# GitHubOfAndrew/TeAMOFlow

Hardware: AMD Instinct MI355X
Metric: train_interactions_per_sec (higher is better)
Workload: dtype f32

## Files before the change

### include/tmf.h

```cpp
#ifndef TMF_H
#define TMF_H

#include <stddef.h>
#include <stdint.h>

#ifdef __cplusplus
extern "C" {
#endif

#define TMF_VERSION 203

#define TMF_OK 0
#define TMF_E_INVALID (-1)
#define TMF_E_LAUNCH (-2)
#define TMF_E_UNSUPPORTED (-3)

#define TMF_EPI_ADAM 0
#define TMF_EPI_GRAD 1

int tmf_version(void);
const char* tmf_last_error(void);

int tmf_padded_ld(int n_components);

// ... 83 lines not shown
    const int64_t* rowptr;
    const int32_t* col;
    const int32_t* pos_off;
    int32_t n_users, n_samples, n_slices;
    int32_t slice_begin, slice_count, item_base;
    int32_t flags;
    int32_t n_items;
} tmf_slice_lists;
#define TMF_SLICE_XCD_MAJOR 1
#define TMF_SLICE_N_ITEMS_STATED 2
int tmf_wmrb_scores3_f32(const tmf_slice_lists* lists, const void* U, const void* V, float* sp, float* p,
                         int n_components, void* stream);
int tmf_wmrb_scores3_bf16(const tmf_slice_lists* lists, const void* U, const void* V, float* sp, float* p,
                          int n_components, void* stream);
int tmf_wmrb_scores5_users_per_workgroup(void);
int tmf_wmrb_scores5_supported(int n_components, int bf16, int64_t n_items);
size_t tmf_wmrb_scores5_workspace_bytes(int64_t n_wg, int32_t n_windows, int wgs_per_launch);
int tmf_wmrb_scores5_f32(const int32_t* ids, const int32_t* outs, const int64_t* wg_ptr, int64_t n_wg, int64_t n_users,
                         int64_t n_items, const void* U, const void* V, float* sp, float* p, int n_components,
                         int wgs_per_launch, const int32_t* wstart, int32_t n_windows, int lag, void* workspace,
                         size_t workspace_bytes, void* stream);
int tmf_wmrb_scores5_bf16(const int32_t* ids, const int32_t* outs, const int64_t* wg_ptr, int64_t n_wg, int64_t n_users,
                          int64_t n_items, const void* U, const void* V, float* sp, float* p, int n_components,
                          int wgs_per_launch, const int32_t* wstart, int32_t n_windows, int lag, void* workspace,
                          size_t workspace_bytes, void* stream);
int tmf_wmrb_scores6_users_per_group(void);
int tmf_wmrb_scores6_supported(int n_components, int bf16, int64_t n_items);
int tmf_wmrb_scores6_f32(const int32_t* ids, const int32_t* outs, const int64_t* chunk_ptr, int64_t n_groups, int32_t n_slices,
                         int64_t n_users, int64_t n_items, const void* U, const void* V, float* sp, float* p, int n_components,
                         void* stream);
int tmf_wmrb_scores6_bf16(const int32_t* ids, const int32_t* outs, const int64_t* chunk_ptr, int64_t n_groups, int32_t n_slices,
                          int64_t n_users, int64_t n_items, const void* U, const void* V, float* sp, float* p, int n_components,
                          void* stream);
int tmf_wmrb_hinge2(const int64_t* rowptr, const float* val, const float* p, const float* sp, int32_t n_users,
                    int32_t n_samples, float c, float* delta, float* D, float* loss_part, void* stream);
int tmf_wmrb_hinge2_ordered(const int64_t* rowptr, const float* val, const float* p, const float* sp, int32_t n_users,
                            int32_t n_samples, float c, float* delta, float* D, float* loss_part, const int32_t* user_order,
                            void* stream);
int tmf_bpr_pairs(const int64_t* rowptr, const float* val, const float* p, const float* sp, int32_t n_users, int32_t n_samples,
                  float* delta, float* D, float* loss_part, const int32_t* user_order, void* stream);
int tmf_wmrb_gradu3_f32(const tmf_slice_lists* lists, const float* D, const float* delta, const void* V, float* part,
                        int per_slice_launches, int n_components, void* stream);
int tmf_wmrb_gradu3_bf16(const tmf_slice_lists* lists, const float* D, const float* delta, const void* V, float* part,
                         int per_slice_launches, int n_components, void* stream);
int tmf_wmrb_gradu4_supported(int n_components, int bf16);
size_t tmf_wmrb_gradu4_workspace_bytes(int32_t n_users, int32_t n_slices, int32_t users_per_launch);
int tmf_wmrb_gradu4_f32(const tmf_slice_lists* lists, const float* D, const float* delta, const void* V, const void* U_old,
                        void* U_out, int n_components, int epi, tmf_adam adam, int32_t users_per_launch, void* workspace,
                        size_t workspace_bytes, void* stream);
int tmf_wmrb_gradu4_bf16(const tmf_slice_lists* lists, const float* D, const float* delta, const void* V, const void* U_old,
                         void* U_out, int n_components, int epi, tmf_adam adam, int32_t users_per_launch, void* workspace,
                         size_t workspace_bytes, void* stream);
int tmf_wmrb_finish_f32(const float* part, int32_t n_slices, int32_t n_users, const void* U_old, void* U_out,
                        int n_components, int epi, tmf_adam adam, void* stream);
int tmf_wmrb_finish_bf16(const float* part, int32_t n_slices, int32_t n_users, const void* U_old, void* U_out,
                         int n_components, int epi, tmf_adam adam, void* stream);

int tmf_adam_fresh_rows_f32(float* W, const float* G, int64_t n_rows, int n_components,
                            tmf_adam adam, void* stream);

int64_t tmf_bias_colsum_part_rows(int64_t n_rows);
int tmf_bias_colsum_f32(const float* G, int64_t n_rows, int n_components, double* part, int64_t part_rows, double* colsum,
                        void* stream);
int tmf_bias_adam_f32(const double* part, int64_t part_rows, float* b, float* g_out, int n_components, tmf_adam adam,
                      void* stream);
int tmf_adam_bias_rows_f32(float* W, const float* G, const float* b_new, float* E, int64_t n_rows, int n_components,
// ... 148 lines not shown
```

### teamoflow_amd/_engine.py

```python
import ctypes
import os

import torch

from . import _lib

DEFAULT_CHUNK = 1024
PART_BUDGET = int(os.environ.get('TMF_PART_BUDGET', 8 << 30))


def row_bytes(n_components, dtype=torch.float32):
    return _lib.padded_ld(n_components, dtype) * (2 if dtype is torch.bfloat16 else 4)


def _excl_cumsum(x):
    out = torch.zeros(x.numel() + 1, dtype=torch.int64, device=x.device)
    torch.cumsum(x, 0, out=out[1:])
    return out


def take_interactions(indices, values, keep, user_offset=0, item_offset=0):
    u = indices[:, 0][keep] - user_offset
    j = indices[:, 1][keep] - item_offset
    return torch.stack([u, j], dim=1), values[keep]
# ... 314 lines not shown
            ws = torch.empty(lib.tmf_wmrb_entry_lists_workspace_bytes(nnz, m, S), dtype=torch.uint8, device=dev)
            _lib.check(lib.tmf_wmrb_entry_lists(_lib.ptr(plan.user_of), _lib.ptr(plan.col_u), _lib.ptr(plan.val_u), nnz,
                                                _lib.ptr(self.R), i32(m), i32(S), i32(n), i32(C), _lib.ptr(self.ent_row),
                                                _lib.ptr(ent_id), _lib.ptr(rowptr), _lib.ptr(ws), ws.numel(),
                                                _lib.stream_ptr()), lib)
            del ws
        else:
            upc = max(1, -(-m // C))
            ku = plan.user_of.to(torch.int64)
            kp = torch.where(plan.val_u > 0, (ku // upc) * n + plan.col_u.to(torch.int64), torch.full_like(ku, C * n))
            ks = (torch.arange(m, dtype=torch.int64) // upc).repeat_interleave(S) * n + self.R.reshape(-1).to(torch.int64)
            keys = torch.cat([kp, ks])
            ent_id = torch.sort(keys, stable=True)[1]
            rowptr = _excl_cumsum(torch.bincount(keys, minlength=C * n + 1))
            owner = torch.cat([ku, torch.arange(m, dtype=torch.int64).repeat_interleave(S)])
            self.ent_row = owner[ent_id].to(torch.int32)
            ent_id = ent_id.to(torch.int32)
        self.rowptr_e = rowptr[:C * n + 1].contiguous()
        self.ent_w = ent_id
        self.rows4 = bool(rows4)
        self.vrows = VirtualRows(self.rowptr_e, C, n) if self.rows4 and os.environ.get('TMF_ROWS5', '1') != '0' else None
        if not item_lists or self.rows4:
            self.seg_e = None
        elif C > 1:
            out_row = torch.arange(C * n, device=dev) % n
            self.seg_e = SegmentTable(self.rowptr_e, chunk, out_row=out_row, n_out=n)
        else:
            self.seg_e = SegmentTable(self.rowptr_e, chunk)
        self.wbuf = torch.zeros(E, dtype=torch.float32, device=dev)
        self.delta = self.wbuf[:nnz]
        self.hinge_order = hinge_user_order(plan.rowptr_u)
        self.D = self.wbuf[nnz:].view(m, S)
        self._lists = None
        self.s5 = self.s6 = None

    def lists(self, plan):
        if self._lists is None:
            m, S = self.R.shape
            self._lists = _lib.SliceLists(self.R.data_ptr(), self.slice_off.data_ptr(), plan.rowptr_u.data_ptr(),
                                          plan.col_u.data_ptr(), self.pos_off.data_ptr(), m, S, self.n_slices, 0, 0, 0,
                                          (_lib.SLICE_XCD_MAJOR if self.xcd_major else 0) | _lib.SLICE_N_ITEMS_STATED, int(plan.n_items))
        return ctypes.byref(self._lists)

    def window_lists(self, plan, slice_begin, slice_count, item_base):
        m, S = self.R.shape
        return _lib.SliceLists(self.R.data_ptr(), self.slice_off.data_ptr(), plan.rowptr_u.data_ptr(), plan.col_u.data_ptr(),
                               self.pos_off.data_ptr(), m, S, self.n_slices, slice_begin, slice_count, item_base,
                               _lib.SLICE_N_ITEMS_STATED, int(plan.n_items))

    def D_in_model_order(self):
        if not self.sliced:
            return self.D
        perm = torch.sort(self.R_model.to(torch.int64), dim=1, stable=True)[1]
        out = torch.empty_like(self.D)
        out.scatter_(1, perm, self.D)
        return out


def row_stationary_wanted(n_users, n_items, n_samples, nnz, n_components, dtype=torch.float32, sliced=True):
    env = os.environ.get('TMF_ROW_STATIONARY')
    if env == '0' or not sliced:
        return False
    if not _lib.load_library().tmf_wmrb_gradu4_supported(int(n_components), int(dtype is torch.bfloat16)):
        return False
    return env == '1' or short_visits(n_users, n_items, n_samples, nnz, n_components, dtype)


# ... 69 lines not shown
        cnt = ptr[1:] - ptr[:-1]
        ptr8 = _excl_cumsum((cnt + 7) // 8 * 8)
        E8 = int(ptr8[-1])
        self.ids = torch.empty(E8 + 8, dtype=i32, device=dev)
        self.outs = torch.full((E8 + 8,), self.PAD, dtype=i32, device=dev)
        self.ids[E8:] = 0
        step = 1 << 27
        for q0 in range(0, E8, step):
            q = torch.arange(q0, min(q0 + step, E8), device=dev, dtype=torch.int64)
            st = torch.searchsorted(ptr8, q, right=True) - 1
            r = q - ptr8[st]
            c = cnt[st]
            src = ptr[st] + torch.minimum(r, c - 1)
            self.ids[q0:q0 + q.numel()] = ids_sorted[src]
            self.outs[q0:q0 + q.numel()] = torch.where(r < c, outs_sorted[src], torch.full_like(src, self.PAD).to(i32))
            del q, st, r, c, src
        self.n_entries, self.n_padded = E, E8
        return ptr8, rowptr


class Scores6Plan(_ScoreStreams):

    def __init__(self, plan, wplan, n_components, dtype=torch.float32, slice_bytes=None):
        lib = _lib.load_library()
        self.key = (int(n_components), dtype)
        UG = int(lib.tmf_wmrb_scores6_users_per_group())
        n = plan.n_items
        self.n_groups = ng = -(-wplan.R.shape[0] // UG)
        slice_bytes = int(os.environ.get('TMF_S6_SLICE_BYTES', slice_bytes or SCORES6_SLICE_BYTES))
        ns = int(min(max(1, -(-n * row_bytes(n_components, dtype) // slice_bytes)), max(1, (2 ** 31 - 1) // max(ng, 1))))
        width = -(-n // ns)
        self.n_slices = ns = -(-n // width)
        self.chunk_ptr, _ = self._build(plan, wplan, UG, lambda grp, item: (item // width) * ng + grp, ns * ng)


def scores5_wanted(plan, wplan, n_components, dtype=torch.float32):
    if os.environ.get('TMF_SCORES5') != '1' or wplan is None or not wplan.sliced or not plan.col_u.is_cuda:
        return False
    m, S = wplan.R.shape
    if m * S >= 2 ** 31 or plan.nnz >= 2 ** 31:
        return False
    return bool(_lib.load_library().tmf_wmrb_scores5_supported(int(n_components), int(dtype is torch.bfloat16), int(plan.n_items)))


class Scores5Plan(_ScoreStreams):

    def __init__(self, plan, wplan, n_components, dtype=torch.float32, slice_bytes=None):
        lib = _lib.load_library()
        dev = plan.col_u.device
        self.key = (int(n_components), dtype)
        UB = int(lib.tmf_wmrb_scores5_users_per_workgroup())
        n = plan.n_items
        self.n_wg = n_wg = -(-wplan.R.shape[0] // UB)
        slice_bytes = int(os.environ.get('TMF_S5_SLICE_BYTES', slice_bytes or (512 << 10)))
        ns = int(min(max(1, -(-n * row_bytes(n_components, dtype) // slice_bytes)), 4096, max(1, (2 ** 31 - 1) // max(n_wg, 1))))
        width = -(-n // ns)
        self.n_slices = ns
        i32 = torch.int32
        self.wg_ptr, rowptr = self._build(plan, wplan, UB, lambda wg, item: wg * ns + item // width, n_wg * ns, keys_per_stream=ns)
        wg_ptr8, wg_ptr = self.wg_ptr, rowptr[::ns]
        every = max(1, int(os.environ.get('TMF_S5_PACE_EVERY', 32)), -(-ns // 4000))
        firsts = list(range(0, ns, every))
        off = rowptr[:n_wg * ns].view(n_wg, ns)[:, firsts] - wg_ptr[:-1, None]
        self.n_windows = nwin = len(firsts) + 1
        self.wstart = torch.zeros(n_wg, nwin + 1, dtype=i32, device=dev)
        self.wstart[:, 1:nwin] = ((off + 7) // 8).to(i32)
# ... 36 lines not shown
        self.feat_v = None if item_feat is None else FeatureSide(item_feat, self._pad(V0, dev), self.r, plan.n_items)
        self.relu_v = None if item_relu is None else ReLUSide(self._pad(V0, dev), self.r, plan.n_items, **item_relu)
        own_v = item_feat is None and item_relu is None
        if V_tables is None:
            self.V = self._pad(V0, dev) if own_v else torch.zeros(plan.n_items, self.ld, dtype=torch.float32, device=dev)
            self.V_nxt = torch.empty_like(self.V) if item_bias is None and own_v else None
        else:
            self.V, self.V_nxt = V_tables
        self.bias_v = None if item_bias is None else BiasSide(self.V, item_bias, self.r)
        self.plan, self.wplan = plan, wplan
        self.l2, self.l2_G = [0.0, 0.0], [None, None]
        need = dict(slab=max(plan.seg_u.n_slab, plan.seg_i.n_slab if plan.seg_i else 0,
                             wplan.seg_e.n_slab if wplan is not None and wplan.seg_e is not None else 0,
                             wplan.vrows.n_slab if wplan is not None and wplan.vrows is not None else 0,
                             *(f.n_slab for f in (self.feat_u, self.feat_v) if f is not None), 1) * self.ld,
                    loss_part=max(plan.seg_u.nseg, plan.n_users, 1))
        need['slab'] = max([need['slab']] + [f.n_slab * f.ld_aux for f in (self.relu_u, self.relu_v) if f is not None])
        self.row_stationary = False
        if wplan is not None and wplan.sliced:
            m, S = wplan.R.shape
            self.row_stationary = row_stationary_wanted(m, plan.n_items, S, plan.nnz, self.r, dtype)
            self.users_per_launch = int(os.environ.get('TMF_G4_USERS', 32768))
            if self.row_stationary:
                nb = _lib.load_library().tmf_wmrb_gradu4_workspace_bytes(m, wplan.n_slices, self.users_per_launch)
                self.g4_sync = torch.zeros(max(nb // 4, 1), dtype=torch.int32, device=dev)
            ns = wplan.n_slices
            if ns * m * self.ld * 4 <= PART_BUDGET:
                self.part_layers, self.gradu_launches = ns, 0
            elif wplan.xcd_major:
                self.part_layers, self.gradu_launches = min(8, ns), 3
            else:
                self.part_layers, self.gradu_launches = 1, 1
            need.update(sp=m * S, pk=max(plan.nnz, 1), part=self.part_layers * max(m, 1) * self.ld)
            if scores6_wanted(plan, wplan, self.r, dtype):
                if wplan.s6 is None or wplan.s6.key != (self.r, dtype):
                    wplan.s6 = Scores6Plan(plan, wplan, self.r, dtype)
            else:
                wplan.s6 = None
            if wplan.seg_e is not None and scores5_wanted(plan, wplan, self.r, dtype):
                if wplan.s5 is None or wplan.s5.key != (self.r, dtype):
                    wplan.s5 = Scores5Plan(plan, wplan, self.r, dtype)
            else:
                wplan.s5 = None
        if wplan is not None and wplan.rows4:
            L = _lib.load_library()
            per_group = L.tmf_wsum_rows4_rows_per_group(self.r, int(dtype is torch.bfloat16))
            if not per_group:
                raise ValueError('the row-stationary item pass needs rows of at least 16 lanes')
            cus = torch.cuda.get_device_properties(dev).multi_processor_count if torch.cuda.is_available() else 256
            self.rows4_per_launch = int(os.environ.get('TMF_ROWS4_PER_LAUNCH', 2 * cus * per_group))
            n_work = wplan.vrows.n_vrows if wplan.vrows is not None else plan.n_items
            nb = L.tmf_wsum_rows4_workspace_bytes(n_work, wplan.user_chunks, self.rows4_per_launch)
            self.rows4_sync = torch.zeros(max(nb // 4, 1), dtype=torch.int32, device=dev)
        self._need = need
        if scratch is None:
            self._bind({k: torch.zeros(v, dtype=torch.float32, device=dev) if k == 'loss_part'
                        else torch.empty(v, dtype=torch.float32, device=dev) for k, v in need.items()})
        else:
            scratch.setdefault('states', []).append(self)
        for side, E in ((self.feat_u, self.U), (self.feat_v, self.V)):
            if side is not None:
                feature_forward(side.plan, side.W, E, self.slab, self.r)
        for side, E in ((self.relu_u, self.U), (self.relu_v, self.V)):
            if side is not None:
                relu_forward(side, E, self.slab)

    def _bind(self, bufs):
# ... 368 lines not shown
                                                       user_epi, adam, wt, s))
    _row_pass_finish(lib, p.seg_u, st.slab, st.U, U_out, r, user_epi, adam, s, st.sfx)
    _lib.check(lib.tmf_sum_f32(_lib.ptr(st.loss_part), p.seg_u.nseg, _lib.ptr(loss_out), s), lib)
    V_out = st.V_nxt if item_out is None else item_out
    _timed(prof, 'logistic_item_pass', lambda: lg_pass(p.seg_i.cstruct(), _lib.ptr(p.row_i), _lib.ptr(p.val_i), _lib.ptr(st.V),
                                                       _lib.ptr(st.U), _lib.ptr(V_out), _lib.ptr(st.slab), None, r, item_epi, adam,
                                                       wt, s))
    _row_pass_finish(lib, p.seg_i, st.slab, st.V, V_out, r, item_epi, adam, s, st.sfx)


def epoch_kl(st, adam, loss_out, item_epi=_lib.EPI_ADAM, item_out=None, prof=None, user_epi=_lib.EPI_ADAM, user_out=None):
    lib, p, r = _lib.get(), st.plan, st.r
    s = _lib.stream_ptr()
    kl_pass = getattr(lib, 'tmf_kl_pass' + st.sfx)
    _timed(prof, 'kl_moments', lambda: getattr(lib, 'tmf_kl_moments' + st.sfx)(
        p.seg_u.cstruct(), _lib.ptr(p.col_u), _lib.ptr(p.val_u), _lib.ptr(st.U), _lib.ptr(st.V), _lib.ptr(st.kl_part), r, s))
    _timed(prof, 'kl_coeffs', lambda: lib.tmf_kl_coeffs(_lib.ptr(st.kl_part), p.seg_u.nseg, _lib.ptr(loss_out), _lib.ptr(st.kl_coef), s))
    U_out = st.U_nxt if user_out is None else user_out
    _timed(prof, 'kl_user_pass', lambda: kl_pass(p.seg_u.cstruct(), _lib.ptr(p.col_u), _lib.ptr(p.val_u), _lib.ptr(st.U), _lib.ptr(st.V),
                                          _lib.ptr(U_out), _lib.ptr(st.slab), _lib.ptr(st.kl_coef), r, user_epi, adam, s))
    _row_pass_finish(lib, p.seg_u, st.slab, st.U, U_out, r, user_epi, adam, s, st.sfx)
    V_out = st.V_nxt if item_out is None else item_out
    _timed(prof, 'kl_item_pass', lambda: kl_pass(p.seg_i.cstruct(), _lib.ptr(p.row_i), _lib.ptr(p.val_i), _lib.ptr(st.V), _lib.ptr(st.U),
                                          _lib.ptr(V_out), _lib.ptr(st.slab), _lib.ptr(st.kl_coef), r, item_epi, adam, s))
    _row_pass_finish(lib, p.seg_i, st.slab, st.V, V_out, r, item_epi, adam, s, st.sfx)


def _wmrb_user_pass_sliced(lib, st, adam, c, prof=None, user_epi=_lib.EPI_ADAM, U_out=None, pairs='hinge'):
    p, w, r = st.plan, st.wplan, st.r
    i32 = ctypes.c_int32
    m, S, ns = p.n_users, w.S, w.n_slices
    s = _lib.stream_ptr()
    lists = w.lists(p)
    s5, s6 = w.s5, w.s6
    if s6 is not None:
        _timed(prof, 'wmrb_scores', lambda: getattr(lib, 'tmf_wmrb_scores6' + st.sfx)(
            _lib.ptr(s6.ids), _lib.ptr(s6.outs), _lib.ptr(s6.chunk_ptr), s6.n_groups, i32(s6.n_slices), m, p.n_items, _lib.ptr(st.U),
            _lib.ptr(st.V), _lib.ptr(st.sp), _lib.ptr(st.pk), r, s))
    elif s5 is not None:
        _timed(prof, 'wmrb_scores', lambda: getattr(lib, 'tmf_wmrb_scores5' + st.sfx)(
            _lib.ptr(s5.ids), _lib.ptr(s5.outs), _lib.ptr(s5.wg_ptr), s5.n_wg, m, p.n_items, _lib.ptr(st.U), _lib.ptr(st.V),
            _lib.ptr(st.sp), _lib.ptr(st.pk), r, s5.wgs_per_launch, _lib.ptr(s5.wstart) if s5.paced else None, i32(s5.n_windows),
            s5.lag, _lib.ptr(s5.sync) if s5.paced else None, s5.sync.numel() * 4, s))
    else:
        _timed(prof, 'wmrb_scores', lambda: getattr(lib, 'tmf_wmrb_scores3' + st.sfx)(lists, _lib.ptr(st.U), _lib.ptr(st.V), _lib.ptr(st.sp),
                                                                                _lib.ptr(st.pk), r, s))
    if pairs == 'bpr':
        _timed(prof, 'bpr_pairs', lambda: lib.tmf_bpr_pairs(_lib.ptr(p.rowptr_u), _lib.ptr(p.val_u), _lib.ptr(st.pk), _lib.ptr(st.sp),
                                                            i32(m), i32(S), _lib.ptr(w.delta), _lib.ptr(w.D), _lib.ptr(st.loss_part),
                                                            _lib.ptr(w.hinge_order), s))
    else:
        _timed(prof, 'wmrb_hinge', lambda: lib.tmf_wmrb_hinge2_ordered(_lib.ptr(p.rowptr_u), _lib.ptr(p.val_u), _lib.ptr(st.pk), _lib.ptr(st.sp),
                                                                i32(m), i32(S), c, _lib.ptr(w.delta), _lib.ptr(w.D), _lib.ptr(st.loss_part),
                                                                _lib.ptr(w.hinge_order), s))
    if st.row_stationary:
        _timed(prof, 'wmrb_gradu', lambda: getattr(lib, 'tmf_wmrb_gradu4' + st.sfx)(
            lists, _lib.ptr(w.D), _lib.ptr(w.delta), _lib.ptr(st.V), _lib.ptr(st.U), _lib.ptr(st.U_nxt if U_out is None else U_out),
            r, user_epi, adam, i32(st.users_per_launch), _lib.ptr(st.g4_sync), st.g4_sync.numel() * 4, s))
        return
    _timed(prof, 'wmrb_gradu', lambda: getattr(lib, 'tmf_wmrb_gradu3' + st.sfx)(
        lists, _lib.ptr(w.D), _lib.ptr(w.delta), _lib.ptr(st.V), _lib.ptr(st.part),
        st.gradu_launches, r, s))
    _timed(prof, 'wmrb_finish', lambda: getattr(lib, 'tmf_wmrb_finish' + st.sfx)(_lib.ptr(st.part), i32(st.part_layers), i32(m),
                                                                          _lib.ptr(st.U), _lib.ptr(st.U_nxt if U_out is None else U_out),
                                                                          r, user_epi, adam, s))


def epoch_wmrb(st, adam, c, loss_out, item_epi=_lib.EPI_ADAM, item_out=None, prof=None, user_epi=_lib.EPI_ADAM, user_out=None,
# ... 39 lines not shown
```

### teamoflow_amd/_lib.py

```python
import ctypes
import os
import subprocess

import torch

_HERE = os.path.dirname(os.path.abspath(__file__))
LIB_PATH = os.environ.get('TMF_LIB', os.path.join(_HERE, 'libtmf.so'))
CSRC = os.path.join(_HERE, 'csrc')

EPI_ADAM, EPI_GRAD = 0, 1


class EngineUnavailable(RuntimeError):
    pass


class EngineError(RuntimeError):
    pass


class Adam(ctypes.Structure):
    _fields_ = [('alpha', ctypes.c_float), ('one_minus_b1', ctypes.c_float), ('one_minus_b2', ctypes.c_float),
                ('eps', ctypes.c_float)]

# ... 35 lines not shown
    'tmf_padded_ld_bf16': (_I, [_I]),
    'tmf_adam_fresh': (Adam, [_F]),
    'tmf_csr_build_workspace_bytes': (_SZ, [_L]),
    'tmf_csr_build': (_I, [_P, _P, _L, _I32, _I32, _P, _P, _P, _P, _P, _SZ, _P]),
    'tmf_stable_order_workspace_bytes': (_SZ, [_L]),
    'tmf_csc_perm': (_I, [_P, _L, _I32, _P, _P, _P, _SZ, _P]),
    'tmf_stable_order_i32': (_I, [_P, _L, _L, _P, _P, _P, _P, _SZ, _P]),
    'tmf_sort_samples_workspace_bytes': (_SZ, [_I32, _I32]),
    'tmf_sort_samples': (_I, [_P, _I32, _I32, _I32, _P, _P, _SZ, _P]),
    'tmf_slice_offsets': (_I, [_P, _P, _L, _I32, _I32, _I32, _P, _P]),
    'tmf_wmrb_entry_lists_workspace_bytes': (_SZ, [_L, _I32, _I32]),
    'tmf_wmrb_entry_lists': (_I, [_P, _P, _P, _L, _P, _I32, _I32, _I32, _I32, _P, _P, _P, _P, _SZ, _P]),
    'tmf_mse_pass_f32': (_I, [_SEG, _P, _P, _P, _P, _P, _P, _P, _I, _I, Adam, _P]),
    'tmf_kl_moments_f32': (_I, [_SEG, _P, _P, _P, _P, _P, _I, _P]),
    'tmf_kl_moments_bf16': (_I, [_SEG, _P, _P, _P, _P, _P, _I, _P]),
    'tmf_kl_coeffs': (_I, [_P, _L, _P, _P, _P]),
    'tmf_kl_pass_f32': (_I, [_SEG, _P, _P, _P, _P, _P, _P, _P, _I, _I, Adam, _P]),
    'tmf_kl_pass_bf16': (_I, [_SEG, _P, _P, _P, _P, _P, _P, _P, _I, _I, Adam, _P]),
    'tmf_logistic_pass_f32': (_I, [_SEG, _P, _P, _P, _P, _P, _P, _P, _I, _I, Adam, _I, _P]),
    'tmf_logistic_pass_bf16': (_I, [_SEG, _P, _P, _P, _P, _P, _P, _P, _I, _I, Adam, _I, _P]),
    'tmf_wsum_pass_f32': (_I, [_SEG, _P, _P, _P, _P, _P, _P, _P, _I, _I, Adam, _P]),
    'tmf_wsum_rows4_rows_per_group': (_I, [_I, _I]),
    'tmf_wsum_rows4_workspace_bytes': (_SZ, [_I32, _I32, _I32]),
    'tmf_wsum_rows4_f32': (_I, [_P, _I32, _I32, _P, _P, _P, _P, _P, _P, _I, _I, Adam, _I32, _P, _SZ, _P]),
    'tmf_wsum_rows5_workspace_bytes': (_SZ, [_I32, _I32, _I32]),
    'tmf_wsum_rows5_f32': (_I, [_P, _I32, _I32, _P, _P, _P, _P, _P, _P, _P, _P, _P, _P, _P, _I32, _I, _I, Adam, _I32, _P, _SZ, _P]),
    'tmf_combine_rows_f32': (_I, [_P, _P, _L, _P, _P, _P, _I, _I, Adam, _P]),
    'tmf_wmrb_user_pass_f32': (_I, [_P, _P, _P, _P, _I32, _I32, _F, _P, _P, _P, _P, _P, _P, _P, _I, _I, Adam, _P]),
    'tmf_wmrb_user_pass_fits': (_I, [_I32, _I]),
    'tmf_wmrb_scores3_f32': (_I, [_SL, _P, _P, _P, _P, _I, _P]),
    'tmf_wmrb_scores6_users_per_group': (_I, []),
    'tmf_wmrb_scores6_supported': (_I, [_I, _I, _L]),
    'tmf_wmrb_scores6_f32': (_I, [_P, _P, _P, _L, _I32, _L, _L, _P, _P, _P, _P, _I, _P]),
    'tmf_wmrb_scores5_users_per_workgroup': (_I, []),
    'tmf_wmrb_scores5_supported': (_I, [_I, _I, _L]),
    'tmf_wmrb_scores5_workspace_bytes': (_SZ, [_L, _I32, _I]),
    'tmf_wmrb_scores5_f32': (_I, [_P, _P, _P, _L, _L, _L, _P, _P, _P, _P, _I, _I, _P, _I32, _I, _P, _SZ, _P]),
    'tmf_wmrb_hinge2': (_I, [_P, _P, _P, _P, _I32, _I32, _F, _P, _P, _P, _P]),
    'tmf_wmrb_hinge2_ordered': (_I, [_P, _P, _P, _P, _I32, _I32, _F, _P, _P, _P, _P, _P]),
    'tmf_bpr_pairs': (_I, [_P, _P, _P, _P, _I32, _I32, _P, _P, _P, _P, _P]),
    'tmf_wmrb_gradu3_f32': (_I, [_SL, _P, _P, _P, _P, _I, _I, _P]),
    'tmf_wmrb_gradu4_supported': (_I, [_I, _I]),
    'tmf_wmrb_gradu4_workspace_bytes': (_SZ, [_I32, _I32, _I32]),
    'tmf_wmrb_gradu4_f32': (_I, [_SL, _P, _P, _P, _P, _P, _I, _I, Adam, _I32, _P, _SZ, _P]),
    'tmf_wmrb_finish_f32': (_I, [_P, _I32, _I32, _P, _P, _I, _I, Adam, _P]),
    'tmf_adam_fresh_rows_f32': (_I, [_P, _P, _L, _I, Adam, _P]),
    'tmf_bias_colsum_part_rows': (_L, [_L]),
    'tmf_bias_colsum_f32': (_I, [_P, _L, _I, _P, _L, _P, _P]),
    'tmf_bias_adam_f32': (_I, [_P, _L, _P, _P, _I, Adam, _P]),
    'tmf_adam_bias_rows_f32': (_I, [_P, _P, _P, _P, _L, _I, Adam, _P]),
    'tmf_feat_pass_f32': (_I, [_SEG, _P, _P, _P, _P, _P, _P, _I, _I, Adam, _P]),
    'tmf_relu_embed_f32': (_I, [_P, _P, _P, _P, _L, _I, _I, _P]),
    'tmf_relu_dhidden_f32': (_I, [_P, _P, _P, _P, _P, _L, _I, _I, _P]),
    'tmf_relu_part_rows': (_L, [_L]),
    'tmf_relu_dweights_f32': (_I, [_P, _P, _P, _P, _L, _L, _I, _I, _P]),
    'tmf_relu_adam_weights_f32': (_I, [_P, _L, _P, _P, _P, _I, _I, Adam, _P]),
    'tmf_adam_step': (Adam, [_F, _I]),
    'tmf_adam_state_rows_f32': (_I, [_P, _P, _P, _P, _L, _I, Adam, _P]),
    'tmf_adam_fresh_rows_l2_f32': (_I, [_P, _P, _L, _I, Adam, _F, _P]),
    'tmf_adam_fresh_rows_l2_bf16': (_I, [_P, _P, _L, _I, Adam, _F, _P]),
    'tmf_adam_state_rows_l2_f32': (_I, [_P, _P, _P, _P, _L, _I, Adam, _F, _P]),
    'tmf_adam_bias_rows_l2_f32': (_I, [_P, _P, _P, _P, _L, _I, Adam, _F, _P]),
    'tmf_mse_pass_bf16': (_I, [_SEG, _P, _P, _P, _P, _P, _P, _P, _I, _I, Adam, _P]),
    'tmf_wsum_rows4_bf16': (_I, [_P, _I32, _I32, _P, _P, _P, _P, _P, _P, _I, _I, Adam, _I32, _P, _SZ, _P]),
    'tmf_wsum_rows5_bf16': (_I, [_P, _I32, _I32, _P, _P, _P, _P, _P, _P, _P, _P, _P, _P, _P, _I32, _I, _I, Adam, _I32, _P, _SZ, _P]),
    'tmf_wsum_pass_bf16': (_I, [_SEG, _P, _P, _P, _P, _P, _P, _P, _I, _I, Adam, _P]),
# ... 121 lines not shown
```

### teamoflow_amd/csrc/tmf_wmrb.hip

```cpp
#include <math.h>
#include <stdlib.h>

#include <type_traits>

#include "tmf_common.h"

namespace tmf {

constexpr int kThreads = 256;
constexpr int kWaves = kThreads / 64;
constexpr int kPosChunk = 512;
constexpr int kUnrollW = 4;
constexpr int kG4Unroll = 4;

__host__ __device__ inline int round4(int x) { return (x + 3) & ~3; }

__host__ __device__ inline int sp_padded(int S) {
    const int nf4 = (S + 3) / 4;
    const int per = ((nf4 + 2 * kWaves - 1) / (2 * kWaves) + 1) & ~1;
    return 4 * 2 * kWaves * per;
}

__device__ __forceinline__ void count_ge0_x4(int& c0, int& c1, float x0, float x1, float x2, float x3) {
    unsigned long long m0, m1, m2, m3;
// ... 1234 lines not shown
template <typename T>
static int wmrb_scores6_impl(const int32_t* ids, const int32_t* outs, const int64_t* chunk_ptr, int64_t n_groups, int32_t n_slices,
                             int64_t n_users, int64_t n_items, const void* U, const void* V, float* sp, float* p, int n_components,
                             void* stream) {
    if (n_users == 0 || n_slices == 0) return TMF_OK;
    const RowGeom geom = row_geom_of<T>(n_components);
    TMF_REQUIRE(ids && outs && chunk_ptr && U && V && sp && p, "wmrb_scores6: null pointer");
    TMF_REQUIRE(n_groups == (n_users + kS6Users - 1) / kS6Users && n_slices > 0, "wmrb_scores6: %lld groups for %lld users (%d per group), %d slices",
                (long long)n_groups, (long long)n_users, kS6Users, n_slices);
    if (!s6_supported(n_components, std::is_same<T, __bf16>::value, n_items)) {
        set_error("wmrb_scores6: needs rows of 32 lanes (fp32 65..128 / bf16 129..256 components) and fewer than 2^24 items in a table "
                  "below 4 GB (got %d components, %lld items)", n_components, (long long)n_items);
        return TMF_E_UNSUPPORTED;
    }
    const int64_t per_slice = n_groups * 64 * kS6Waves;
    const int max_slices = (int)((((int64_t)1 << 32) - 1) / per_slice);
    TMF_REQUIRE(max_slices >= 1, "wmrb_scores6: %lld user groups exceed one launch", (long long)n_groups);
    for (int s0 = 0; s0 < n_slices; s0 += max_slices) {
        const int nsl = (n_slices - s0 < max_slices) ? n_slices - s0 : max_slices;
        const unsigned blocks = (unsigned)(n_groups * nsl);
#define CALL(G_, NV_)                                                                                                       \
    {                                                                                                                       \
        if constexpr (G_ == 32) {                                                                                           \
            hipLaunchKernelGGL((k_wmrb_scores6<NV_, T>), dim3(blocks), dim3(64 * kS6Waves), 0, (hipStream_t)stream, ids, outs, \
                               chunk_ptr, (int64_t)s0 * n_groups, n_groups, n_users, (const T*)U, (const T*)V, sp, p);      \
        }                                                                                                                   \
    }
        TMF_DISPATCH(T, geom, CALL);
#undef CALL
    }
    return check_launch("tmf_wmrb_scores6");
}

static int s5_launches(int64_t n_wg, int wgs_per_launch) { return (int)((n_wg + wgs_per_launch - 1) / wgs_per_launch); }
static int s5_wgs_per_launch(int wgs_per_launch) {
    if (wgs_per_launch > 0) return wgs_per_launch;
    int dev = 0, cus = 256;
    if (hipGetDevice(&dev) == hipSuccess) (void)hipDeviceGetAttribute(&cus, hipDeviceAttributeMultiprocessorCount, dev);
    return cus > 0 ? cus : 256;
}

template <typename T>
static int wmrb_scores5_impl(const int32_t* ids, const int32_t* outs, const int64_t* wg_ptr, int64_t n_wg, int64_t n_users,
                             int64_t n_items, const void* U, const void* V, float* sp, float* p, int n_components,
                             int wgs_per_launch, const int32_t* wstart, int32_t n_windows, int lag, void* workspace,
                             size_t workspace_bytes, void* stream) {
    if (n_wg == 0 || n_users == 0) return TMF_OK;
    const RowGeom geom = row_geom_of<T>(n_components);
    TMF_REQUIRE(ids && outs && wg_ptr && U && V && sp && p, "wmrb_scores5: null pointer");
    TMF_REQUIRE(n_wg == (n_users + kS5Users - 1) / kS5Users, "wmrb_scores5: %lld workgroups for %lld users (%d per workgroup)",
                (long long)n_wg, (long long)n_users, kS5Users);
    const size_t row_bytes = (size_t)geom.ld * sizeof(T);
    if (geom.G != 32 || row_bytes * kS5Users > 128 * 1024 || n_items <= 0 || n_items >= (1 << 24) ||
        (int64_t)n_items * (int64_t)row_bytes >= ((int64_t)1 << 32)) {
        set_error("wmrb_scores5: needs rows of 32 lanes (fp32 65..128 / bf16 129..256 components) and fewer than 2^24 items "
                  "in a table below 4 GB (got %d components, %lld items)", n_components, (long long)n_items);
        return TMF_E_UNSUPPORTED;
    }
    wgs_per_launch = s5_wgs_per_launch(wgs_per_launch);
    const int launches = s5_launches(n_wg, wgs_per_launch);
    const bool paced = wstart != nullptr && workspace != nullptr && n_windows > 1;
    const size_t per_launch = (size_t)8 * (paced ? n_windows : 0) * kS5Stride * sizeof(int);
    if (paced) {
        TMF_REQUIRE(n_windows <= kS5MaxWindows && lag >= 0, "wmrb_scores5: %d windows (at most %d), lag %d", n_windows, kS5MaxWindows, lag);
        TMF_REQUIRE(workspace_bytes >= per_launch * launches, "wmrb_scores5: workspace of %zu bytes needed, got %zu", per_launch * launches,
                    workspace_bytes);
// ... 51 lines not shown
                                          int64_t n_users, int64_t n_items, const void* U, const void* V, float* sp,      \
                                          float* p, int n_components, int wgs_per_launch, const int32_t* wstart,          \
                                          int32_t n_windows, int lag, void* workspace, size_t workspace_bytes,            \
                                          void* stream) {                                                                 \
        return wmrb_scores5_impl<T_>(ids, outs, wg_ptr, n_wg, n_users, n_items, U, V, sp, p, n_components, wgs_per_launch, \
                                     wstart, n_windows, lag, workspace, workspace_bytes, stream);                         \
    }                                                                                                                     \
    extern "C" int tmf_wmrb_scores6_##SFX(const int32_t* ids, const int32_t* outs, const int64_t* chunk_ptr, int64_t n_groups, \
                                          int32_t n_slices, int64_t n_users, int64_t n_items, const void* U, const void* V, \
                                          float* sp, float* p, int n_components, void* stream) {                          \
        return wmrb_scores6_impl<T_>(ids, outs, chunk_ptr, n_groups, n_slices, n_users, n_items, U, V, sp, p, n_components, stream); \
    }                                                                                                                     \
    extern "C" int tmf_wmrb_gradu3_##SFX(const tmf_slice_lists* lists, const float* D, const float* delta,                \
                                         const void* V, float* part, int per_slice_launches, int n_components,            \
                                         void* stream) {                                                                  \
        return wmrb_gradu3_impl<T_>(lists, D, delta, V, part, per_slice_launches, n_components, stream);                  \
    }                                                                                                                     \
    extern "C" int tmf_wmrb_gradu4_##SFX(const tmf_slice_lists* lists, const float* D, const float* delta, const void* V,  \
                                         const void* U_old, void* U_out, int n_components, int epi, tmf_adam adam,       \
                                         int32_t users_per_launch, void* workspace, size_t workspace_bytes, void* stream) { \
        return wmrb_gradu4_impl<T_>(lists, D, delta, V, U_old, U_out, n_components, epi, adam, users_per_launch, workspace, \
                                    workspace_bytes, stream);                                                            \
    }                                                                                                                     \
    extern "C" int tmf_wmrb_finish_##SFX(const float* part, int32_t n_slices, int32_t n_users, const void* U_old,         \
                                         void* U_out, int n_components, int epi, tmf_adam adam, void* stream) {           \
        return wmrb_finish_impl<T_>(part, n_slices, n_users, U_old, U_out, n_components, epi, adam, stream);               \
    }

TMF_SLICED_ENTRY_POINTS(f32, float)
TMF_SLICED_ENTRY_POINTS(bf16, __bf16)

extern "C" int tmf_wmrb_scores6_users_per_group(void) { return tmf::kS6Users; }
extern "C" int tmf_wmrb_scores6_supported(int n_components, int bf16, int64_t n_items) { return s6_supported(n_components, bf16, n_items); }
extern "C" int tmf_wmrb_scores5_users_per_workgroup(void) { return tmf::kS5Users; }
extern "C" size_t tmf_wmrb_scores5_workspace_bytes(int64_t n_wg, int32_t n_windows, int wgs_per_launch) {
    if (n_wg <= 0 || n_windows <= 1) return 0;
    return (size_t)s5_launches(n_wg, s5_wgs_per_launch(wgs_per_launch)) * 8 * (size_t)n_windows * tmf::kS5Stride * sizeof(int);
}
extern "C" int tmf_wmrb_scores5_supported(int n_components, int bf16, int64_t n_items) {
    const tmf::RowGeom geom = bf16 ? tmf::row_geom_bf16(n_components) : tmf::row_geom(n_components);
    const int64_t row_bytes = (int64_t)geom.ld * (bf16 ? 2 : 4);
    return geom.G == 32 && row_bytes * tmf::kS5Users <= 128 * 1024 && n_items > 0 && n_items < (1 << 24) &&
           n_items * row_bytes < ((int64_t)1 << 32);
}
```

Baseline: 1.176 billion.

## Add scores7 kernel that reuses each item row across up to four users

Adds a new WMRB scoring kernel, scores7. It stages 256 user rows in LDS and processes precomputed steps that group up to four users sharing the same item within a sub-chunk. Each V row gathered from global memory is then dotted against several users, and results are buffered in LDS slots before being scattered to sp/p. It is meant to cut redundant item-row gathers compared with scores6, at the cost of a heavy host-side planning pass, extra index memory and large LDS use that limits occupancy. It is enabled automatically when a share heuristic predicts enough items are shared within a group.

```diff
diff --git a/include/tmf.h b/include/tmf.h
--- a/include/tmf.h
+++ b/include/tmf.h
@@ -139,6 +139,12 @@
 int tmf_wmrb_scores6_bf16(const int32_t* ids, const int32_t* outs, const int64_t* chunk_ptr, int64_t n_groups, int32_t n_slices,
                           int64_t n_users, int64_t n_items, const void* U, const void* V, float* sp, float* p, int n_components,
                           void* stream);
+int tmf_wmrb_scores7_users_per_group(void);
+int tmf_wmrb_scores7_slots(void);
+int tmf_wmrb_scores7_supported(int n_components, int bf16, int64_t n_items);
+int tmf_wmrb_scores7_f32(const void* steps, const int32_t* place, const int64_t* sub_step, const int64_t* sub_place,
+                         const int32_t* chunk_sub, int64_t n_groups, int32_t n_slices, int64_t n_users, int64_t n_items,
+                         const void* U, const void* V, float* sp, float* p, int n_components, void* stream);
 int tmf_wmrb_hinge2(const int64_t* rowptr, const float* val, const float* p, const float* sp, int32_t n_users,
                     int32_t n_samples, float c, float* delta, float* D, float* loss_part, void* stream);
 int tmf_wmrb_hinge2_ordered(const int64_t* rowptr, const float* val, const float* p, const float* sp, int32_t n_users,
diff --git a/teamoflow_amd/_engine.py b/teamoflow_amd/_engine.py
--- a/teamoflow_amd/_engine.py
+++ b/teamoflow_amd/_engine.py
@@ -370,7 +370,7 @@
         self.hinge_order = hinge_user_order(plan.rowptr_u)
         self.D = self.wbuf[nnz:].view(m, S)
         self._lists = None
-        self.s5 = self.s6 = None
+        self.s5 = self.s6 = self.s7 = None
 
     def lists(self, plan):
         if self._lists is None:
@@ -506,6 +506,114 @@
         width = -(-n // ns)
         self.n_slices = ns = -(-n // width)
         self.chunk_ptr, _ = self._build(plan, wplan, UG, lambda grp, item: (item // width) * ng + grp, ns * ng)
+
+
+SCORES7_SLICE_BYTES = 4 << 20
+SCORES7_MIN_SHARE = 1.5
+
+
+def scores7_wanted(plan, wplan, n_components, dtype=torch.float32):
+    env = os.environ.get('TMF_SCORES7')
+    if env == '0' or wplan is None or not wplan.sliced or not plan.col_u.is_cuda:
+        return False
+    m, S = wplan.R.shape
+    if m * S >= 2 ** 31 or plan.nnz >= 2 ** 31:
+        return False
+    lib = _lib.load_library()
+    if not lib.tmf_wmrb_scores7_supported(int(n_components), int(dtype is torch.bfloat16), int(plan.n_items)):
+        return False
+    if env == '1':
+        return True
+    if os.environ.get('TMF_SCORES5') == '1' or os.environ.get('TMF_SCORES6') == '1':
+        return False
+    if plan.n_items * row_bytes(n_components, dtype) < 8 * VISIT_SLICE_BYTES:
+        return False
+    UG = int(lib.tmf_wmrb_scores7_users_per_group())
+    return UG * (S + plan.nnz / max(m, 1)) / plan.n_items >= SCORES7_MIN_SHARE
+
+
+class Scores7Plan:
+
+    K = 4
+
+    def __init__(self, plan, wplan, n_components, dtype=torch.float32, slice_bytes=None, slots=None):
+        lib = _lib.load_library()
+        self.key = (int(n_components), dtype)
+        dev, i32, i64, K = plan.col_u.device, torch.int32, torch.int64, self.K
+        self.users_per_group = UG = int(lib.tmf_wmrb_scores7_users_per_group())
+        self.pad_slot = cap = int(lib.tmf_wmrb_scores7_slots())
+        self.slots = SL = max(1, min(cap, int(os.environ.get('TMF_S7_SLOTS', slots or cap))))
+        m, S = wplan.R.shape
+        n, nnz = plan.n_items, plan.nnz
+        E = nnz + m * S
+        self.n_groups = ng = -(-m // UG)
+        slice_bytes = int(os.environ.get('TMF_S7_SLICE_BYTES', slice_bytes or SCORES7_SLICE_BYTES))
+        ns = int(min(max(1, -(-n * row_bytes(n_components, dtype) // slice_bytes)), max(1, (2 ** 31 - 1) // max(ng, 1))))
+        self.width = width = -(-n // ns)
+        self.n_slices = ns = -(-n // width)
+        nc = ns * ng
+        ar = torch.arange(E, device=dev, dtype=i64)
+        user = torch.cat([plan.user_of.to(i64), torch.arange(m, device=dev, dtype=i64).repeat_interleave(S)])
+        item = torch.cat([plan.col_u.to(i64), wplan.R.reshape(-1).to(i64)])
+        lu = (user % UG).to(i32)
+        chunk = (item // width) * ng + user // UG
+        del user
+        ordA = torch.sort((chunk * width + item % width) * UG + lu, stable=True)[1]
+        chunkA = chunk[ordA]
+        cnt_c = torch.bincount(chunk, minlength=nc)
+        del chunk
+        chunk_sub = _excl_cumsum((cnt_c + SL - 1) // SL)
+        subA = chunk_sub[chunkA] + (ar - _excl_cumsum(cnt_c)[chunkA]) // SL
+        del chunkA, cnt_c
+        self.n_sub = n_sub = int(chunk_sub[-1])
+        self.chunk_sub = chunk_sub.to(i32)
+        self.sub_place = sub_place = _excl_cumsum(torch.bincount(subA, minlength=n_sub))
+        sub_e = torch.empty(E, dtype=i64, device=dev)
+        sub_e[ordA] = subA
+        ordB = torch.sort(sub_e * UG + lu, stable=True)[1]
+        place_e = torch.cat([-1 - torch.arange(nnz, device=dev, dtype=i32), torch.arange(m * S, device=dev, dtype=i32)])
+        self.place = place_e[ordB]
+        del place_e
+        slot_e = torch.empty(E, dtype=i32, device=dev)
+        slot_e[ordB] = (ar - sub_place[sub_e[ordB]]).to(i32)
+        del sub_e, ordB
+        slotA, itemA, luA = slot_e[ordA], item[ordA].to(i32), lu[ordA]
+        del slot_e, item, lu, ordA
+        new_run = torch.ones(E, dtype=torch.bool, device=dev)
+        if E > 1:
+            new_run[1:] = (subA[1:] != subA[:-1]) | (itemA[1:] != itemA[:-1])
+        run_start = torch.nonzero(new_run).flatten()
+        run_of = torch.cumsum(new_run, 0) - 1
+        del new_run
+        run_len = torch.diff(run_start, append=torch.tensor([E], device=dev, dtype=i64))
+        run_steps = (run_len + K - 1) // K
+        del run_len
+        run_step0 = _excl_cumsum(run_steps)
+        self.n_steps = n_steps = int(run_step0[-1])
+        sub_steps = torch.zeros(n_sub, dtype=i64, device=dev)
+        sub_steps.scatter_add_(0, subA[run_start], run_steps)
+        self.sub_step = _excl_cumsum(sub_steps)
+        del subA, sub_steps, run_steps
+        pos = ar - run_start[run_of]
+        del ar, run_start
+        stepA = run_step0[run_of] + pos // K
+        k = pos % K
+        del pos, run_of, run_step0
+        users = torch.zeros(n_steps, K, dtype=i64, device=dev)
+        slot4 = torch.full((n_steps, K), cap, dtype=i64, device=dev)
+        first = k == 0
+        users[stepA[first]] = luA[first].to(i64)[:, None]
+        users[stepA, k] = luA.to(i64)
+        slot4[stepA, k] = slotA.to(i64)
+        steps = torch.zeros(n_steps + 1, 4, dtype=i32, device=dev)
+        steps[stepA[first], 0] = itemA[first]
+        del first, stepA, k, luA, slotA, itemA
+        w = users[:, 0] | (users[:, 1] << 8) | (users[:, 2] << 16) | (users[:, 3] << 24)
+        steps[:n_steps, 1] = torch.where(w >= 2 ** 31, w - 2 ** 32, w).to(i32)
+        steps[:n_steps, 2] = (slot4[:, 0] | (slot4[:, 1] << 16)).to(i32)
+        steps[:n_steps, 3] = (slot4[:, 2] | (slot4[:, 3] << 16)).to(i32)
+        self.steps = steps
+        self.n_entries = E
 
 
 def scores5_wanted(plan, wplan, n_components, dtype=torch.float32):
@@ -608,7 +716,18 @@
             else:
                 self.part_layers, self.gradu_launches = 1, 1
             need.update(sp=m * S, pk=max(plan.nnz, 1), part=self.part_layers * max(m, 1) * self.ld)
-            if scores6_wanted(plan, wplan, self.r, dtype):
+            if scores7_wanted(plan, wplan, self.r, dtype):
+                if wplan.s7 is None or wplan.s7.key != (self.r, dtype):
+                    if os.environ.get('TMF_SCORES7') == '1':
+                        wplan.s7 = Scores7Plan(plan, wplan, self.r, dtype)
+                    else:
+                        try:
+                            wplan.s7 = Scores7Plan(plan, wplan, self.r, dtype)
+                        except torch.OutOfMemoryError:
+                            wplan.s7 = None
+            else:
+                wplan.s7 = None
+            if wplan.s7 is None and scores6_wanted(plan, wplan, self.r, dtype):
                 if wplan.s6 is None or wplan.s6.key != (self.r, dtype):
                     wplan.s6 = Scores6Plan(plan, wplan, self.r, dtype)
             else:
@@ -1043,8 +1162,12 @@
     m, S, ns = p.n_users, w.S, w.n_slices
     s = _lib.stream_ptr()
     lists = w.lists(p)
-    s5, s6 = w.s5, w.s6
-    if s6 is not None:
+    s5, s6, s7 = w.s5, w.s6, w.s7
+    if s7 is not None:
+        _timed(prof, 'wmrb_scores', lambda: lib.tmf_wmrb_scores7_f32(
+            _lib.ptr(s7.steps), _lib.ptr(s7.place), _lib.ptr(s7.sub_step), _lib.ptr(s7.sub_place), _lib.ptr(s7.chunk_sub), s7.n_groups,
+            i32(s7.n_slices), m, p.n_items, _lib.ptr(st.U), _lib.ptr(st.V), _lib.ptr(st.sp), _lib.ptr(st.pk), r, s))
+    elif s6 is not None:
         _timed(prof, 'wmrb_scores', lambda: getattr(lib, 'tmf_wmrb_scores6' + st.sfx)(
             _lib.ptr(s6.ids), _lib.ptr(s6.outs), _lib.ptr(s6.chunk_ptr), s6.n_groups, i32(s6.n_slices), m, p.n_items, _lib.ptr(st.U),
             _lib.ptr(st.V), _lib.ptr(st.sp), _lib.ptr(st.pk), r, s))
diff --git a/teamoflow_amd/_lib.py b/teamoflow_amd/_lib.py
--- a/teamoflow_amd/_lib.py
+++ b/teamoflow_amd/_lib.py
@@ -91,6 +91,10 @@
     'tmf_wmrb_scores6_users_per_group': (_I, []),
     'tmf_wmrb_scores6_supported': (_I, [_I, _I, _L]),
     'tmf_wmrb_scores6_f32': (_I, [_P, _P, _P, _L, _I32, _L, _L, _P, _P, _P, _P, _I, _P]),
+    'tmf_wmrb_scores7_users_per_group': (_I, []),
+    'tmf_wmrb_scores7_slots': (_I, []),
+    'tmf_wmrb_scores7_supported': (_I, [_I, _I, _L]),
+    'tmf_wmrb_scores7_f32': (_I, [_P, _P, _P, _P, _P, _L, _I32, _L, _L, _P, _P, _P, _P, _I, _P]),
     'tmf_wmrb_scores5_users_per_workgroup': (_I, []),
     'tmf_wmrb_scores5_supported': (_I, [_I, _I, _L]),
     'tmf_wmrb_scores5_workspace_bytes': (_SZ, [_L, _I32, _I]),
diff --git a/teamoflow_amd/csrc/tmf_wmrb.hip b/teamoflow_amd/csrc/tmf_wmrb.hip
--- a/teamoflow_amd/csrc/tmf_wmrb.hip
+++ b/teamoflow_amd/csrc/tmf_wmrb.hip
@@ -1290,6 +1290,177 @@
     return check_launch("tmf_wmrb_scores6");
 }
 
+namespace tmf {
+constexpr int kS7Users = 256;
+constexpr int kS7Slots = 6144;
+constexpr int kS7K = 4;
+constexpr int kS7Waves = 16;
+constexpr int kS7Flight = 2;
+constexpr uint32_t kS7RowBytes = 512;
+constexpr size_t kS7Lds = (size_t)kS7Users * kS7RowBytes + (size_t)(kS7Slots + 64) * sizeof(float);
+
+struct S7Streams {
+    const int4* steps;
+    const int32_t* place;
+    const int64_t* sub_step;
+    const int64_t* sub_place;
+    const int32_t* chunk_sub;
+};
+
+__global__ __launch_bounds__(64 * kS7Waves) void k_wmrb_scores7(S7Streams a, int64_t chunk0, int64_t n_groups, int64_t n_users,
+                                                                const float* __restrict__ U, const float* __restrict__ V,
+                                                                float* __restrict__ sp, float* __restrict__ p) {
+    constexpr int NG = 8 * kS7Waves, NT = 64 * kS7Waves, FL = kS7Flight;
+    extern __shared__ __attribute__((aligned(16))) char smem_raw[];
+    float* sbuf = reinterpret_cast<float*>(smem_raw + (size_t)kS7Users * kS7RowBytes);
+    const int tid = threadIdx.x, lane = tid & 63, g = lane & 7, gid = tid >> 3;
+    const int64_t chunk = chunk0 + blockIdx.x;
+    const int sub_b = a.chunk_sub[chunk], sub_e = a.chunk_sub[chunk + 1];
+    if (sub_b == sub_e) return;
+    const int64_t ubeg = (chunk % n_groups) * kS7Users;
+    const int nu = (int)((n_users - ubeg < kS7Users) ? n_users - ubeg : kS7Users);
+    {
+        const tmf_f4* src = reinterpret_cast<const tmf_f4*>(reinterpret_cast<const char*>(U) + ubeg * (int64_t)kS7RowBytes);
+        tmf_f4* dst = reinterpret_cast<tmf_f4*>(smem_raw);
+        for (int i = tid; i < nu * (int)(kS7RowBytes / 16); i += NT) dst[i] = __builtin_nontemporal_load(src + i);
+    }
+    __syncthreads();
+    const uint32_t par = (lane >> 4) & 1;
+    const uint32_t offA = 16u * g + 128u * par, offB = 16u * g + 128u * (par ^ 1u);
+    struct Row {
+        float4 v[4];
+    };
+    auto dot = [](const Row& x, const Row& y) {
+        float q[4];
+#pragma unroll
+        for (int v = 0; v < 4; ++v) {
+            tmf_f2 a = tmf_f2{x.v[v].x, x.v[v].y} * tmf_f2{y.v[v].x, y.v[v].y};
+            a = __builtin_elementwise_fma(tmf_f2{x.v[v].z, x.v[v].w}, tmf_f2{y.v[v].z, y.v[v].w}, a);
+            q[v] = a.x + a.y;
+        }
+        return (q[0] + q[2]) + (q[1] + q[3]);
+    };
+    for (int sub = sub_b; sub < sub_e; ++sub) {
+        const int64_t st0 = a.sub_step[sub];
+        const int nsteps = (int)(a.sub_step[sub + 1] - st0);
+        const int64_t pl0 = a.sub_place[sub];
+        const int nslots = (int)(a.sub_place[sub + 1] - pl0);
+        const int4* rec0 = a.steps + st0;
+        const int mine = nsteps > gid ? (nsteps - gid + NG - 1) / NG : 0;
+        const int rounds = __builtin_amdgcn_readfirstlane(mine);
+        const int32_t* pl = a.place + pl0;
+        int32_t where[kS7Slots / NT];
+#pragma unroll
+        for (int q = 0; q < kS7Slots / NT; ++q) where[q] = (tid + NT * q < nslots) ? __builtin_nontemporal_load(pl + tid + NT * q) : 0;
+        if (rounds > 0) {
+            auto fetch = [&](int i) {
+                const int st = gid + NG * i;
+                return rec0[st < nsteps ? st : nsteps - 1];
+            };
+            auto gather = [&](Row& y, const int4& r) {
+                const char* base = reinterpret_cast<const char*>(V);
+                const uint32_t oa = row_byte_off<kS7RowBytes>((uint32_t)r.x, offA), ob = row_byte_off<kS7RowBytes>((uint32_t)r.x, offB);
+                y.v[0] = *reinterpret_cast<const float4*>(base + oa);
+                y.v[1] = *reinterpret_cast<const float4*>(base + ob);
+                y.v[2] = *reinterpret_cast<const float4*>(base + oa + 256);
+                y.v[3] = *reinterpret_cast<const float4*>(base + ob + 256);
+            };
+            auto finish = [&](const Row& y, const int4& r, int i) {
+                float s[kS7K];
+#pragma unroll
+                for (int k = 0; k < kS7K; ++k) {
+                    const uint32_t lu = ((uint32_t)r.y >> (8 * k)) & 0xffu;
+                    const char* xa = smem_raw + (lu * kS7RowBytes + offA);
+                    const char* xb = smem_raw + (lu * kS7RowBytes + offB);
+                    Row x;
+                    x.v[0] = *reinterpret_cast<const float4*>(xa);
+                    x.v[1] = *reinterpret_cast<const float4*>(xb);
+                    x.v[2] = *reinterpret_cast<const float4*>(xa + 256);
+                    x.v[3] = *reinterpret_cast<const float4*>(xb + 256);
+                    float t = dot(x, y);
+                    t += TMF_DPP_MOV(t, 0xB1);
+                    t += TMF_DPP_MOV(t, 0x4E);
+                    t += TMF_DPP_MOV(t, 0x141);
+                    s[k] = t;
+                }
+                const float mine_s = (g & 2) ? ((g & 1) ? s[3] : s[2]) : ((g & 1) ? s[1] : s[0]);
+                const uint32_t w = (g & 2) ? (uint32_t)r.w : (uint32_t)r.z;
+                uint32_t slot = (g & 1) ? (w >> 16) : (w & 0xffffu);
+                slot = (slot < (uint32_t)kS7Slots && gid + NG * i < nsteps) ? slot : (uint32_t)kS7Slots;
+                if (g < kS7K) sbuf[slot] = mine_s;
+            };
+            Row y[FL];
+            int4 rec[2 * FL];
+#pragma unroll
+            for (int j = 0; j < FL; ++j) rec[j] = fetch(j);
+#pragma unroll
+            for (int j = 0; j < FL; ++j) {
+                gather(y[j], rec[j]);
+                rec[FL + j] = fetch(FL + j);
+            }
+            int i = 0;
+            for (; i + 2 * FL <= rounds; i += 2 * FL) {
+#pragma unroll
+                for (int j = 0; j < 2 * FL; ++j) {
+                    __builtin_amdgcn_sched_barrier(0);
+                    finish(y[j % FL], rec[j], i + j);
+                    __builtin_amdgcn_sched_barrier(0);
+                    gather(y[j % FL], rec[(j + FL) % (2 * FL)]);
+                    rec[j] = fetch(i + j + 2 * FL);
+                }
+            }
+            const int rem = rounds - i;
+#pragma unroll
+            for (int j = 0; j < 2 * FL - 1; ++j) {
+                if (j < rem) {
+                    __builtin_amdgcn_sched_barrier(0);
+                    finish(y[j % FL], rec[j], i + j);
+                    __builtin_amdgcn_sched_barrier(0);
+                    if (j + FL < rem) gather(y[j % FL], rec[j + FL]);
+                }
+            }
+        }
+        __syncthreads();
+#pragma unroll
+        for (int q = 0; q < kS7Slots / NT; ++q)
+            if (tid + NT * q < nslots)
+                __builtin_nontemporal_store(sbuf[tid + NT * q], where[q] >= 0 ? sp + where[q] : p + ~where[q]);
+        __syncthreads();
+    }
+}
+
+}
+
+static bool s7_supported(int n_components, int bf16, int64_t n_items) {
+    return !bf16 && n_components >= 65 && n_components <= 128 && s6_supported(n_components, 0, n_items);
+}
+
+static int wmrb_scores7_impl(const void* steps, const int32_t* place, const int64_t* sub_step, const int64_t* sub_place,
+                             const int32_t* chunk_sub, int64_t n_groups, int32_t n_slices, int64_t n_users, int64_t n_items,
+                             const void* U, const void* V, float* sp, float* p, int n_components, void* stream) {
+    if (n_users == 0 || n_slices == 0) return TMF_OK;
+    TMF_REQUIRE(steps && place && sub_step && sub_place && chunk_sub && U && V && sp && p, "wmrb_scores7: null pointer");
+    TMF_REQUIRE(n_groups == (n_users + kS7Users - 1) / kS7Users && n_slices > 0, "wmrb_scores7: %lld groups for %lld users (%d per group), %d slices",
+                (long long)n_groups, (long long)n_users, kS7Users, n_slices);
+    if (!s7_supported(n_components, 0, n_items)) {
+        set_error("wmrb_scores7: needs fp32 rows of 65..128 components and fewer than 2^24 items in a table below 4 GB "
+                  "(got %d components, %lld items)", n_components, (long long)n_items);
+        return TMF_E_UNSUPPORTED;
+    }
+    static LdsGrant grant;
+    if (int rc = grant_dynamic_lds(reinterpret_cast<const void*>(&k_wmrb_scores7), kS7Lds, grant)) return rc;
+    const S7Streams a{static_cast<const int4*>(steps), place, sub_step, sub_place, chunk_sub};
+    const int64_t per_slice = n_groups * 64 * kS7Waves;
+    const int max_slices = (int)((((int64_t)1 << 32) - 1) / per_slice);
+    TMF_REQUIRE(max_slices >= 1, "wmrb_scores7: %lld user groups exceed one launch", (long long)n_groups);
+    for (int s0 = 0; s0 < n_slices; s0 += max_slices) {
+        const int nsl = (n_slices - s0 < max_slices) ? n_slices - s0 : max_slices;
+        hipLaunchKernelGGL(k_wmrb_scores7, dim3((unsigned)(n_groups * nsl)), dim3(64 * kS7Waves), kS7Lds, (hipStream_t)stream, a,
+                           (int64_t)s0 * n_groups, n_groups, n_users, (const float*)U, (const float*)V, sp, p);
+    }
+    return check_launch("tmf_wmrb_scores7");
+}
+
 static int s5_launches(int64_t n_wg, int wgs_per_launch) { return (int)((n_wg + wgs_per_launch - 1) / wgs_per_launch); }
 static int s5_wgs_per_launch(int wgs_per_launch) {
     if (wgs_per_launch > 0) return wgs_per_launch;
@@ -1407,6 +1578,15 @@
 
 extern "C" int tmf_wmrb_scores6_users_per_group(void) { return tmf::kS6Users; }
 extern "C" int tmf_wmrb_scores6_supported(int n_components, int bf16, int64_t n_items) { return s6_supported(n_components, bf16, n_items); }
+extern "C" int tmf_wmrb_scores7_f32(const void* steps, const int32_t* place, const int64_t* sub_step, const int64_t* sub_place,
+                                    const int32_t* chunk_sub, int64_t n_groups, int32_t n_slices, int64_t n_users, int64_t n_items,
+                                    const void* U, const void* V, float* sp, float* p, int n_components, void* stream) {
+    return wmrb_scores7_impl(steps, place, sub_step, sub_place, chunk_sub, n_groups, n_slices, n_users, n_items, U, V, sp, p,
+                             n_components, stream);
+}
+extern "C" int tmf_wmrb_scores7_users_per_group(void) { return tmf::kS7Users; }
+extern "C" int tmf_wmrb_scores7_slots(void) { return tmf::kS7Slots; }
+extern "C" int tmf_wmrb_scores7_supported(int n_components, int bf16, int64_t n_items) { return s7_supported(n_components, bf16, n_items); }
 extern "C" int tmf_wmrb_scores5_users_per_workgroup(void) { return tmf::kS5Users; }
 extern "C" size_t tmf_wmrb_scores5_workspace_bytes(int64_t n_wg, int32_t n_windows, int wgs_per_launch) {
     if (n_wg <= 0 || n_windows <= 1) return 0;
```

After: 1.273 billion, median of 6. +8.3%, better.
